# dcherednik/atracdenc

Hardware: AMD Instinct MI355X
Metric: ATRAC3 1024-sample stereo frames/sec (higher is better)
Workload: dtype f32; 1 GPU; ATRAC3 LP2 132 kbps stereo, 64 streams x 64 frames = 4096 frames per GPU per step (BASELINE configs[1]), 'noise' PCM resident in HBM, frames written to HBM (PCIe excluded); streams_per_gpu=64, frame_bytes=384, input=noise, tonal_components=True, parallelism=streams/1, launch=1 process x 1 GPU(s), one host thread and one at3hip context per device, collectives=none (no RCCL); start/stop barrier only

## Files before the change

### atracdenc_amd/csrc/at3_k_backend.hpp

```cpp
#pragma once
#include "at3_bits.hpp"
#include "at3_common.hpp"

namespace at3 {

struct BackParams {
    float* specs;
    const float* ges;
    const Curve* curves;
    PsyRec* psy;
    float* loud;
    float* loud_state;
    uint8_t* out;
    int n_blocks;
    int f0;
    int n_streams;
    int no_tonal;
    int js;
    int frame_sz;
    int bfu_idx_const;
    int mono_js;
    struct QuantRec* quant;
    int flat_literal;
    unsigned long long* counters;
// ... 132 lines not shown
        __syncthreads();
        if (wave > 0) {
            if (k + 2 < kLoudChunks) {
                loud_produce(s_t[k & 1], s_curve, s_ges, u, k + 2, xa);
                if (k + 4 < kLoudChunks) loud_request(p.specs, c0, n_cf, u, k + 4, xa);
            }
        } else if (chain) {
            loud_consume(s_t[(k + 1) & 1] + lane * kLoudRow, l);
        }
        __syncthreads();
    }
    if (chain && c0 + lane < n_cf) p.psy[c0 + lane].loud_ch = l;
}

constexpr int kPsyCf = 4;
__device__ __forceinline__ bool psy_flat_job(int wave, int lane, int& k, int& b)
{
    if (wave == 0) { k = lane / 3; b = 26 + lane % 3; return lane < 12; }
    if (wave == 1) { k = lane / 10; b = 16 + lane % 10; return lane < 40; }
    if (wave == 2) { k = lane / 8; b = 8 + lane % 8; return lane < 32; }
    k = 0; b = 8;
    return false;
}
__device__ __forceinline__ bool psy_scale_job(int wave, int lane, int& k, int& b)
{
    if (wave == 0) { k = lane / 6; b = 26 + lane % 6; return lane < 24; }
    if (wave == 1) { k = lane / 10; b = 16 + lane % 10; return lane < 40; }
    if (wave == 2) { k = lane / 16; b = lane % 16; return true; }
    k = 0; b = 0;
    return false;
}

__device__ __attribute__((noinline)) float flatness_literal_wave(const Libm64* M, const float* sp, int len, double arith, int lane)
{
    const double floor_ = (double)1e-12f;
    double lg = 0.0;
    if (lane < len) {
// ... 34 lines not shown
        float4 x4[kPsyCf];
#pragma unroll
        for (int k = 0; k < kPsyCf; ++k) x4[k] = *reinterpret_cast<const float4*>(specs0 + (size_t)(k < ncf ? k : 0) * 1024 + 4 * tid);
#pragma unroll
        for (int k = 0; k < kPsyCf; ++k) *reinterpret_cast<float4*>(s_spec[k] + 4 * tid) = (k < ncf) ? x4[k] : float4{0.0f, 0.0f, 0.0f, 0.0f};
    }
    if (tid < 32 * kPsyCf) {
        (&s_run_len[0][0])[tid] = 0;
        const int k = tid >> 5, b = tid & 31;
        if (k < ncf && (p.no_tonal || b < 8 || b > 28)) rec0[k].flat[b] = 0.0f;
    }
    if (tid < kPsyCf) s_any[tid] = 0;
    if (tid >= 128 && tid < 192) s_scale[tid - 128] = scale_v;
    __syncthreads();

    int fk, fb;
    const bool flat_job = !p.no_tonal && psy_flat_job(wave, lane, fk, fb) && fk < ncf;
    float flat = 1.0f;
    double arith = 0.0;
    bool want_literal = false;
    if (flat_job) {
        const int b = fb;
        const float* sp = s_spec[fk];
        const int start = bfu_start(b), end = bfu_start(b + 1), len = end - start;
        double prod = 1.0;
        int esum = 0;
        const double floor_ = (double)1e-12f;
        for (int i0 = start; i0 < end; i0 += 8) {
            const float4 xa = *reinterpret_cast<const float4*>(sp + i0), xb = *reinterpret_cast<const float4*>(sp + i0 + 4);
            const float ev[8] = {xa.x * xa.x, xa.y * xa.y, xa.z * xa.z, xa.w * xa.w, xb.x * xb.x, xb.y * xb.y, xb.z * xb.z, xb.w * xb.w};
#pragma unroll
            for (int k = 0; k < 8; ++k) {
                const double e = (double)fmaxf(0.0f, ev[k]);
                arith += e;
                const double d = e > floor_ ? e : floor_;
                const uint64_t bits = (uint64_t)__double_as_longlong(d);
                esum += (int)((bits >> 52) & 0x7ffu) - 1022;
                prod *= __longlong_as_double((long long)((bits & 0x800fffffffffffffull) | 0x3fe0000000000000ull));
            }
        }
        arith /= (double)len;
        if (!(arith <= floor_)) {
            const double meanLog = (log(prod) + (double)esum * 0.69314718055994530942) / (double)len;
            const double ratio = exp(meanLog) / arith;
            const float f_lo = (float)fmin(1.0, fmax(0.0, ratio * (1.0 - 1e-12)));
            const float f_hi = (float)fmin(1.0, fmax(0.0, ratio * (1.0 + 1e-12)));
            flat = f_lo;
            want_literal = f_lo != f_hi || p.flat_literal;
        }
    }
    for (unsigned long long rem = __ballot(want_literal); rem; rem &= rem - 1ull) {
        const int src = __builtin_ctzll(rem);
        const int jk = __builtin_amdgcn_readlane(fk, src), jb = __builtin_amdgcn_readlane(fb, src);
        const uint64_t ab = (uint64_t)__double_as_longlong(arith);
        const uint64_t as = (uint64_t)(uint32_t)__builtin_amdgcn_readlane((int)(uint32_t)ab, src) |
// ... 580 lines not shown
```

### atracdenc_amd/csrc/at3_k_gain.hpp

```cpp
#pragma once
#include "at3_common.hpp"

namespace at3 {

struct GainParams {
    const float* sub;
    GainRec* rec;
    cpx* bins;
    BandState* state;
    Curve* curves;
    int n_blocks;
    int f0;
    int js;
    int n_streams;
    int literal;
};

constexpr int kLowCutBin = 38;

__device__ inline void median3_32(const float* in, float* out)
{
    for (int i = 0; i < 32; ++i) {
        const int lo = i > 0 ? i - 1 : 0;
        const int hi = i < 31 ? i + 1 : 31;
// ... 755 lines not shown
        float m[8] = {ma.x, ma.y, ma.z, ma.w, mb.x, mb.y, mb.z, mb.w};
#pragma unroll
        for (int i = 1; i < 8; ++i) {
#pragma unroll
            for (int k = i; k > 0; --k) {
                const float lo = fminf(m[k - 1], m[k]), hi = fmaxf(m[k - 1], m[k]);
                m[k - 1] = lo;
                m[k] = hi;
            }
        }
        rec->lo[sf] = m[2];
        rec->hi[sf] = m[6];
    }
}

__global__ __launch_bounds__(256) void k_gain_tail(GainParams p, int n_items)
{
    __shared__ float s_g[8][32], s_f[8][32], s_m[8][32];
    const int tid = threadIdx.x, grp = tid >> 5, j = tid & 31, half = grp & 1;
    const int nfr = p.n_blocks - p.f0;
    int item = blockIdx.x * 8 + grp;
    const bool valid = item < n_items;
    if (!valid) item = n_items - 1;
    int wg = item;
    const int band = wg % 3; wg /= 3;
    const int ch = wg % 2; wg /= 2;
    const int f = p.f0 + wg % nfr;
    const int s = wg / nfr;
    GainRec* rec = p.rec + (((size_t)s * p.n_blocks + f) * 2 + ch) * 3 + band;
    const float hfr = rec->hfr;
    const float g_j = rec->gain[j];
    asm volatile("" ::"v"(g_j));
    const bool active = valid && !(hfr < 0.05f);
    if (__ballot(active) == 0ull) return;
    float* s_gain = s_g[grp];
    float* s_filt = s_f[grp];
    float* s_minv = s_m[grp];
    const float in_j = active ? g_j : 0.0f;
    s_gain[j] = in_j;
    wave_sync();
    float filt_j;
    {
        const float a = s_gain[j > 0 ? j - 1 : 0], c = s_gain[j < 31 ? j + 1 : 31];
        if (j == 0) filt_j = fmaxf(in_j, c);
        else if (j == 31) filt_j = fmaxf(a, in_j);
        else filt_j = fmaxf(fminf(a, in_j), fminf(fmaxf(a, in_j), c));
    }
    s_filt[j] = filt_j;
    wave_sync();
    s_minv[j] = (j <= 29) ? fminf(fminf(filt_j, s_filt[j < 30 ? j + 1 : 31]), s_filt[j < 30 ? j + 2 : 31]) : -1.0f;
    wave_sync();
    float maxRaw = 0.0f, sum = 0.0f, bestLevel = 0.0f;
    int bestEnd = -1;
    for (int k = 0; k < 32; ++k) {
        const float g = s_gain[k];
        maxRaw = fmaxf(maxRaw, g);
        sum += g;
        const float mv = s_minv[k];
        if (k <= 29 && mv > bestLevel) {
            bestLevel = mv;
            bestEnd = k + 2;
        }
    }
    const uint32_t ge = (uint32_t)(__ballot(filt_j >= bestLevel) >> (32 * half));
    const uint32_t high = (uint32_t)(__ballot(in_j >= bestLevel * 0.7f) >> (32 * half));
    const float last = s_gain[31];
    float plateau = 0.0f;
    bool release = false;
    if (!(bestLevel < 1e-6f)) {
        plateau = bestLevel;
        const uint32_t x = (bestEnd + 1 < 32) ? (ge >> (bestEnd + 1)) : 0u;
        bestEnd += (x == 0xffffffffu) ? 32 : __builtin_ctz(~x);
        if (bestEnd < 31) {
            if (last < bestLevel * 0.1f) release = true;
            else release = ((high >> (bestEnd + 1)) == 0u) && (last < bestLevel * 0.5f);
        }
    }
    const bool usePlateau = plateau > 1e-6f && !release && plateau >= maxRaw * 0.4f;
    if (active && j == 0) {
        rec->cur_hpf = sum / 32.0f;
        rec->target = usePlateau ? plateau : last;
    }
}

constexpr int kScanChunk = 512;
__global__ __launch_bounds__(64) void k_gain_scan(GainParams p, int n_streams)
{
    __shared__ float s_hfr[kScanChunk], s_g31[kScanChunk], s_tgt[kScanChunk], s_hpf[kScanChunk];
    const int lane = threadIdx.x;
    const int idx = blockIdx.x;
    if (idx >= n_streams * 6) return;
    const int band = idx % 3, ch = (idx / 3) % 2, s = idx / 6;
    BandState* st = p.state + (size_t)s * 8 + ch * 4 + band;
    float lvl = st->last_level, tgt = st->last_target, hpf = st->last_hpf;
    const int nfr = p.n_blocks - p.f0;
    for (int base = 0; base < nfr; base += kScanChunk) {
        const int cnt = (nfr - base < kScanChunk) ? nfr - base : kScanChunk;
        for (int i = lane; i < cnt; i += 64) {
            const GainRec* rec = p.rec + (((size_t)s * p.n_blocks + p.f0 + base + i) * 2 + ch) * 3 + band;
            s_hfr[i] = rec->hfr;
            s_g31[i] = rec->gain[31];
            s_tgt[i] = rec->target;
            s_hpf[i] = rec->cur_hpf;
        }
        __syncthreads();
        if (lane == 0) {
            for (int i = 0; i < cnt; ++i) {
                const float h = s_hfr[i], g = s_g31[i], t = s_tgt[i], e = s_hpf[i];
                s_g31[i] = lvl;
                s_tgt[i] = tgt;
                s_hpf[i] = hpf;
                if (h < 0.05f) {
                    lvl = 0.0f;
                } else {
                    lvl = g;
                    tgt = t;
                    hpf = e;
                }
            }
        }
        __syncthreads();
        for (int i = lane; i < cnt; i += 64) {
            GainRec* rec = p.rec + (((size_t)s * p.n_blocks + p.f0 + base + i) * 2 + ch) * 3 + band;
            rec->ctx_level = s_g31[i];
            rec->ctx_target = s_tgt[i];
            rec->ctx_hpf = s_hpf[i];
        }
        __syncthreads();
    }
    if (lane == 0) {
        st->last_level = lvl;
        st->last_target = tgt;
        st->last_hpf = hpf;
    }
}

__device__ inline uint32_t first_set_bit(uint32_t x)
{
    return x ? 31u - (uint32_t)__builtin_clz(x) : 0u;
}

__device__ inline int relation_to_idx(float x)
{
// ... 18 lines not shown

__device__ __forceinline__ float grp_readlane_f(float v, int idx, int half)
{
    const int a = __builtin_amdgcn_readlane((int)__float_as_uint(v), idx);
    const int b = __builtin_amdgcn_readlane((int)__float_as_uint(v), 32 + idx);
    return __uint_as_float((uint32_t)(half ? b : a));
}
__device__ __forceinline__ int grp_readlane_i(int v, int idx, int half)
{
    const int a = __builtin_amdgcn_readlane(v, idx);
    const int b = __builtin_amdgcn_readlane(v, 32 + idx);
    return half ? b : a;
}

struct CurvePts {
    int n;
    int level[7];
    int loc[7];
};


__device__ __forceinline__ void early_mismatch_score_pair(const Log2fTab* L2, const float* gain_interp, float in_j, float in_next, float target,
                                                          const CurvePts& cpA, const CurvePts& cpB, float* s_tmpA, uint8_t* s_ptsA,
                                                          float* aB, float* sqB, float* ltB, uint8_t* s_ptsB, int j, float& scoreA, float& scoreB)
{
    auto cell_div = [&](const CurvePts& cp) -> float {
        uint64_t lo = (uint64_t)(uint32_t)cp.n, hi = 0;
#pragma unroll
        for (int i = 0; i < 7; ++i) {
            lo |= (uint64_t)((uint32_t)cp.level[i] & 0xffu) << (8 * (i + 1));
            hi |= (uint64_t)((uint32_t)cp.loc[i] & 0xffu) << (8 * i);
        }
        float d[8];
        cell_divisors_packed(lo, hi, gain_interp, 8 * j, d);
        float dsum = 0.0f;
#pragma unroll
        for (int k = 0; k < 8; ++k) dsum += d[k];
        return dsum / 8.0f;
    };
    (void)s_ptsA; (void)s_ptsB;
    const float divA = cell_div(cpA), divB = cell_div(cpB);
    int maxLocA = 0, maxLocB = 0;
#pragma unroll
    for (int i = 0; i < 7; ++i) {
        if (i < cpA.n && cpA.loc[i] > maxLocA) maxLocA = cpA.loc[i];
        if (i < cpB.n && cpB.loc[i] > maxLocB) maxLocB = cpB.loc[i];
    }
    int evalA = maxLocA + 3 > 3 ? maxLocA + 3 : 3, evalB = maxLocB + 3 > 3 ? maxLocB + 3 : 3;
    if (evalA > 32) evalA = 32;
    if (evalB > 32) evalB = 32;
    const float eps = 1e-9f;
    const float modA = in_j / fmaxf(divA, eps), modB = in_j / fmaxf(divB, eps);
    const float eA = at3_log2f(L2, fmaxf(modA, eps) / fmaxf(target, eps)), eB = at3_log2f(L2, fmaxf(modB, eps) / fmaxf(target, eps));
    const float sqA = eA * eA, sqvB = eB * eB;
    const float aA = at3_log2f(L2, fmaxf(divA, eps)), avB = at3_log2f(L2, fmaxf(divB, eps));
    s_tmpA[j] = aA;
    aB[j] = avB;
    wave_sync();
    const float aA_next = s_tmpA[j < 31 ? j + 1 : 31], aB_next = aB[j < 31 ? j + 1 : 31];
    wave_sync();
    const float dA = aA_next - aA, dB = aB_next - avB;
    const float w = 0.5f * (in_j + in_next);
    const float ltermA = dA * dA * w, ltermB = dB * dB * w;
    float* st = s_tmpA + 32;
    st[j] = j < evalA ? sqA : 0.0f;
    st[32 + j] = j + 1 < evalA ? ltermA : 0.0f;
    st[64 + j] = j + 1 < evalA ? w : 0.0f;
    sqB[j] = j < evalB ? sqvB : 0.0f;
    ltB[j] = j + 1 < evalB ? ltermB : 0.0f;
    s_tmpA[j] = j + 1 < evalB ? w : 0.0f;
    wave_sync();
    float fitA = 0.0f, leakA = 0.0f, wsumA = 0.0f, fitB = 0.0f, leakB = 0.0f, wsumB = 0.0f;
    {
        const float4* a4 = reinterpret_cast<const float4*>(st);
        const float4* s4 = reinterpret_cast<const float4*>(sqB);
        const float4* l4 = reinterpret_cast<const float4*>(ltB);
        const float4* w4 = reinterpret_cast<const float4*>(s_tmpA);
#pragma unroll
        for (int q = 0; q < 8; ++q) {
            const float4 va = a4[q], vl = a4[8 + q], vw = a4[16 + q], vb = s4[q], vm = l4[q], vx = w4[q];
            const float v[4] = {va.x, va.y, va.z, va.w};
            const float lt[4] = {vl.x, vl.y, vl.z, vl.w};
            const float ww[4] = {vw.x, vw.y, vw.z, vw.w};
            const float vB[4] = {vb.x, vb.y, vb.z, vb.w};
            const float lB[4] = {vm.x, vm.y, vm.z, vm.w};
            const float wB[4] = {vx.x, vx.y, vx.z, vx.w};
#pragma unroll
            for (int t = 0; t < 4; ++t) {
                fitA += v[t];
                leakA += lt[t];
                wsumA += ww[t];
                fitB += vB[t];
                leakB += lB[t];
                wsumB += wB[t];
            }
        }
    }
    wave_sync();
    fitA /= (float)evalA;
    fitB /= (float)evalB;
    if (wsumA > eps) leakA /= wsumA;
    if (wsumB > eps) leakB /= wsumB;
    scoreA = (target <= 1e-9f) ? 0.0f : fitA + 0.25f * leakA;
    scoreB = (target <= 1e-9f) ? 0.0f : fitB + 0.25f * leakB;
}

__global__ __launch_bounds__(256) void k_gain_curve(GainParams p, const Tables* T, int n_streams)
{
    __shared__ float s_in[8][32];
    __shared__ __attribute__((aligned(16))) float s_filt[8][32];
    __shared__ __attribute__((aligned(16))) float s_tmp[8][128];
    __shared__ __attribute__((aligned(16))) int s_tloc[8][32];
    __shared__ __attribute__((aligned(16))) int s_tdelta[8][32];
    __shared__ int s_tlev[8][32];
    __shared__ uint8_t s_pts[8][16];
    __shared__ uint8_t s_pts2[8][16];
    __shared__ Log2fTab s_l2[4];
    __shared__ float s_gi4[4][32];
    const int tid = threadIdx.x;
    const int grp = tid >> 5, j = tid & 31, half = grp & 1;
    const Log2fTab* L2 = &s_l2[tid >> 6];
    const float* gi = s_gi4[tid >> 6];
    const int nfr = p.n_blocks - p.f0;
    const int n_items = n_streams * nfr * 6;
    int item = blockIdx.x * 8 + grp;
    const bool valid = item < n_items;
    if (!valid) item = n_items - 1;
    int idx = item;
    const int band = idx % 3; idx /= 3;
    const int ch = idx % 2; idx /= 2;
    const int f = p.f0 + idx % nfr;
// ... 15 lines not shown
    {
        const float a = s_in[grp][j > 0 ? j - 1 : 0], c = s_in[grp][j < 31 ? j + 1 : 31];
        if (j == 0) filt_j = fmaxf(in_j, c);
        else if (j == 31) filt_j = fmaxf(a, in_j);
        else filt_j = fmaxf(fminf(a, in_j), fminf(fmaxf(a, in_j), c));
    }
    const float in_next = s_in[grp][j < 31 ? j + 1 : 31];
    s_filt[grp][j] = filt_j;
    float maxGain = fmaxf(0.0f, in_j);
#pragma unroll
    for (int m = 1; m < 32; m <<= 1) maxGain = fmaxf(maxGain, __shfl_xor(maxGain, m, 64));
    wave_sync();

    const bool active = valid && !(hfr < 0.05f) && !(target < 1e-6f) && !(savedLastLevel < 1e-6f);
    if (__ballot(active) == 0ull) {
        if (valid && j == 0) {
            Curve out;
            out.pad = 0;
            out.n = 0;
#pragma unroll
            for (int i = 0; i < 7; ++i) {
                out.level[i] = 0;
                out.loc[i] = 0;
            }
            *dst = out;
        }
        return;
    }
    const float intraRatio = maxGain / fmaxf(target, 1e-9f);
    float interRatio = 1.0f;
    if (prevTarget > 1e-6f) interRatio = fmaxf(prevTarget, target) / fmaxf(fminf(prevTarget, target), 1e-9f);
    const bool sticky = intraRatio <= 7.0f && interRatio <= 10.0f;
    const int raw = relation_to_idx(filt_j / target);
    if (__ballot(active && j <= 30 && raw != 4) == 0ull) {
        if (valid && j == 0) {
            Curve out;
            out.pad = 0;
            out.n = 0;
#pragma unroll
            for (int i = 0; i < 7; ++i) {
                out.level[i] = 0;
                out.loc[i] = 0;
            }
            *dst = out;
        }
        return;
    }
    int minIdx = 0, maxIdx = 0;
    {
        float ratioLo = lo_j / target, ratioHi = hi_j / target;
        if (ratioLo > ratioHi) {
            const float t = ratioLo;
            ratioLo = ratioHi;
            ratioHi = t;
        }
        const int idxLo = relation_to_idx(ratioLo), idxHi = relation_to_idx(ratioHi);
        minIdx = idxLo < idxHi ? idxLo : idxHi;
        maxIdx = idxLo < idxHi ? idxHi : idxLo;
    }
    int L = raw;
// ... 2 lines not shown
        if (__ballot(may_stick) != 0ull) {
            for (int round = 0; round < 32; ++round) {
                const int prev = __builtin_amdgcn_update_dpp(0, L, 0x138, 0xf, 0xf, false);
                const int d = raw - prev;
                const int nl = (may_stick && (d == 1 || d == -1) && prev >= minIdx && prev <= maxIdx) ? prev : raw;
                const bool moved = nl != L;
                L = nl;
                if (__ballot(moved) == 0ull) break;
            }
        }
    }
    const unsigned long long nzm = __ballot(active && j <= 30 && L != 4);
    const uint32_t gm = (uint32_t)(nzm >> (32 * half));
    const int targetSf = gm ? 32 - __builtin_clz(gm) : 0;
    float bs = 1.0f;
    if (j >= 1) {
        float leftMax = 0.0f, rightMax = 0.0f;
        for (int i = (j - 3 > 0 ? j - 3 : 0); i < j; ++i) leftMax = fmaxf(leftMax, s_filt[grp][i]);
        for (int i = j; i < (j + 3 < 32 ? j + 3 : 32); ++i) rightMax = fmaxf(rightMax, s_filt[grp][i]);
        const float eps = 1e-9f;
        bs = fmaxf((rightMax + eps) / (leftMax + eps), (leftMax + eps) / (rightMax + eps));
    }
    int nt = 0;
    {
        int prev = 4;
        uint32_t remaining = targetSf >= 31 ? 0x7fffffffu : ((1u << targetSf) - 1u);
        for (int it = 0; it < 32; ++it) {
            const unsigned long long m = __ballot(L != prev);
            const uint32_t cand = (uint32_t)(m >> (32 * half)) & remaining;
            const bool done = cand == 0u;
            if (__ballot(!done) == 0ull) break;
            const int sf = done ? 0 : 31 - __builtin_clz(cand);
            const int lev = __builtin_amdgcn_ds_bpermute(4 * (32 * half + sf), L);
            const float sc = __uint_as_float((uint32_t)__builtin_amdgcn_ds_bpermute(4 * (32 * half + sf + 1), (int)__float_as_uint(bs)));
            if (!done) {
                const int loc = sf + 1;
// ... 30 lines not shown
            }
        }
        const bool keep_t = has_t && ahead < 6;
        const uint32_t kept = (uint32_t)(__ballot(keep_t) >> (32 * half));
        const int pos = j < 31 ? __popc(kept >> (j + 1)) : 0;
        wave_sync();
        if (keep_t) {
            s_tlev[grp][pos] = my_lev;
            s_tloc[grp][pos] = my_loc;
        }
        nt = __popc(kept);
    }
    wave_sync();
    if (nt > 6) nt = 6;
    CurvePts pts;
    pts.n = (active && targetSf > 0) ? nt : 0;
#pragma unroll
    for (int i = 0; i < 7; ++i) {
        pts.level[i] = (i < pts.n) ? s_tlev[grp][i] : 0;
        pts.loc[i] = (i < pts.n) ? s_tloc[grp][i] : 0;
    }
    const bool have = pts.n > 0;
    if (__ballot(have) == 0ull) {
        if (valid && j == 0) {
            Curve out;
            out.pad = 0;
            out.n = 0;
#pragma unroll
            for (int i = 0; i < 7; ++i) {
                out.level[i] = 0;
                out.loc[i] = 0;
            }
            *dst = out;
        }
        return;
    }

    {
        const int wv = tid >> 6, ln = tid & 63;
        const double l2v = (&T->log2f_tab[0][0])[ln < 36 ? ln : 35];
        const float giv = T->gain_interp[(ln & 31) < 31 ? (ln & 31) : 30];
        if (ln < 36) reinterpret_cast<double*>(&s_l2[wv])[ln] = l2v;
        if (ln < 32) s_gi4[wv][ln] = giv;
        wave_sync();
    }
    if (maxGain < 1e-4f) pts.n = 0;
    if (hfr < 0.3f) pts.n = 0;
    const CurvePts before = pts;
    bool changed = false;
    float hpfRmsNextMod = 0.0f;
    bool validMod = false;
    {
        const int nBefore = (pts.n > 0) ? pts.loc[0] : 32;
        float sum = 0.0f;
        for (int sf = 0; sf < 32; ++sf) {
            const float v = s_in[grp][sf];
            if (sf < nBefore) sum += v;
        }
        if (pts.n > 0 && pts.loc[0] > 0) {
            hpfRmsNextMod = (sum / (float)nBefore) / gain_level_of(pts.level[0]);
            validMod = true;
        } else if (pts.n == 0) {
            hpfRmsNextMod = sum / 32;
            validMod = true;
        }
    }
    const bool p0ok = validMod && prevTarget > 1e-6f && hpfRmsNextMod > 1e-6f;
    if (p0ok) {
        const int p0 = relation_to_idx_hdr(prevTarget / hpfRmsNextMod);
        int it = -1;
#pragma unroll
        for (int i = 6; i >= 0; --i)
            if (i < pts.n && pts.loc[i] == 0) it = i;
        if (it >= 0) {
#pragma unroll
            for (int i = 0; i < 7; ++i)
                if (i == it && pts.level[i] != p0) {
                    pts.level[i] = p0;
                    changed = true;
                }
        } else if (p0 != 4 || pts.n > 0) {
#pragma unroll
            for (int i = 6; i > 0; --i) {
                pts.level[i] = pts.level[i - 1];
                pts.loc[i] = pts.loc[i - 1];
            }
            pts.level[0] = p0;
            pts.loc[0] = 0;
            pts.n++;
            changed = true;
        }
    }
    float scoreBefore, scoreAfter;
    early_mismatch_score_pair(L2, gi, in_j, in_next, target, before, pts, s_tmp[grp], s_pts[grp], s_filt[grp], reinterpret_cast<float*>(s_tloc[grp]),
                              reinterpret_cast<float*>(s_tdelta[grp]), s_pts2[grp], j, scoreBefore, scoreAfter);
    scoreBefore = __uint_as_float((uint32_t)opaque_lane_value((int)__float_as_uint(scoreBefore)));
    scoreAfter = __uint_as_float((uint32_t)opaque_lane_value((int)__float_as_uint(scoreAfter)));
    if (changed) {
        bool keepByBoundary = false;
        if (p0ok) {
            const float x = prevTarget / hpfRmsNextMod;
            const float desired = fminf(fmaxf(x, gain_level_of(15)), gain_level_of(0));
            const float scaleBefore = gain_level_of(before.n == 0 ? 4 : before.level[0]);
            const float scaleAfter = gain_level_of(pts.n == 0 ? 4 : pts.level[0]);
            const float eps = 1e-9f;
            const float errBefore = fabsf(at3_log2f(L2, fmaxf(scaleBefore, eps) / fmaxf(desired, eps)));
            const float errAfter = fabsf(at3_log2f(L2, fmaxf(scaleAfter, eps) / fmaxf(desired, eps)));
            keepByBoundary = (errAfter + 0.20f < errBefore);
        }
        if (!keepByBoundary && scoreAfter > scoreBefore * (1.0f + 0.02f)) pts = before;
    }
    if (pts.n >= 2 && pts.loc[0] == 0 && pts.level[0] == pts.level[1]) {
#pragma unroll
        for (int i = 1; i < 7; ++i) {
            pts.level[i - 1] = pts.level[i];
            pts.loc[i - 1] = pts.loc[i];
        }
        pts.n--;
    }
    if (valid && j == 0) {
        Curve out;
        out.pad = 0;
        out.n = (uint8_t)(have ? pts.n : 0);
#pragma unroll
        for (int i = 0; i < 7; ++i) {
            const bool on = have && i < pts.n;
            out.level[i] = (uint8_t)(on ? pts.level[i] : 0);
            out.loc[i] = (uint8_t)(on ? pts.loc[i] : 0);
        }
        *dst = out;
    }
}

}
```

### atracdenc_amd/csrc/at3hip.hip

```cpp
#include <hip/hip_runtime.h>

#include <stdio.h>
#include <stdlib.h>
#include <string.h>

#include <new>

#include "../../include/at3hip.h"
#include "at3_common.hpp"
#include "at3_host_util.hpp"
#include "at3_k_backend.hpp"
#include "at3_k_alloc.hpp"
#include "at3_k_frontend.hpp"
#include "at3_k_front2.hpp"
#include "at3_k_gain.hpp"

using namespace at3;
using at3host::dev_alloc;
using at3host::fail;

namespace {

const struct {
    uint32_t bitrate;
// ... 1189 lines not shown
    float* d_out = nullptr;
    const size_t nb = (size_t)n * 256 * sizeof(float);
    if (hipMalloc((void**)&d_cv, (size_t)n * sizeof(Curve)) != hipSuccess || hipMalloc((void**)&d_out, 2 * nb) != hipSuccess) return AT3HIP_EDEVICE;
    int rc = AT3HIP_OK;
    if (hipMemcpy(d_cv, curves, (size_t)n * sizeof(Curve), hipMemcpyHostToDevice) != hipSuccess) rc = AT3HIP_EDEVICE;
    if (rc == AT3HIP_OK) {
        hipLaunchKernelGGL(k_debug_cell_divisors, dim3((unsigned)((n + 1) / 2)), dim3(64), 0, c->stream, d_cv, c->d_tables, d_out, d_out + (size_t)n * 256, n);
        if (hipStreamSynchronize(c->stream) != hipSuccess || hipMemcpy(out_packed, d_out, nb, hipMemcpyDeviceToHost) != hipSuccess ||
            hipMemcpy(out_ref, d_out + (size_t)n * 256, nb, hipMemcpyDeviceToHost) != hipSuccess)
            rc = AT3HIP_EDEVICE;
    }
    (void)hipFree(d_cv);
    (void)hipFree(d_out);
    return rc;
}
#endif

#include "at3_decoder_host.hpp"
#include "at3_decode.hpp"

struct at3hip_decoder : at3host::DecoderBase {
    at3hip_decoder_config cfg;
    Dec3Tables* d_tables = nullptr;
    float* d_raw = nullptr;
    Dec3Gains* d_gains = nullptr;
};

namespace {

__attribute__((optnone, noinline)) bool build_dec3_tables(Dec3Tables* t)
// ... 137 lines not shown
```

Before: 15.51 million frames/s.

## Split flatness sums across lanes and replace shared-memory gain reductions with DPP/ballot

Psy flatness computation now splits each band's energy and log-product accumulation into 16-element chunks across several lanes, combines them with DPP row shuffles, and falls back to a serial sum only when the exponent range makes summation order matter. k_gain_tail replaces shared-memory median/min/max scans with lane permutes, DPP max reductions and ballots. k_gain_scan replaces the single-lane serial carry with a ballot-based parallel scan per 64 frames. CurvePts is packed into two 64-bit words to cut register shuffling. The changes aim to reduce serial per-lane work and LDS traffic, at the cost of added complexity and a rounding-sensitive fallback path; a debug kernel for the flat sums is also added.

```diff
diff --git a/atracdenc_amd/csrc/at3_k_backend.hpp b/atracdenc_amd/csrc/at3_k_backend.hpp
--- a/atracdenc_amd/csrc/at3_k_backend.hpp
+++ b/atracdenc_amd/csrc/at3_k_backend.hpp
@@ -170,13 +170,93 @@
 }
 
 constexpr int kPsyCf = 4;
-__device__ __forceinline__ bool psy_flat_job(int wave, int lane, int& k, int& b)
-{
-    if (wave == 0) { k = lane / 3; b = 26 + lane % 3; return lane < 12; }
-    if (wave == 1) { k = lane / 10; b = 16 + lane % 10; return lane < 40; }
-    if (wave == 2) { k = lane / 8; b = 8 + lane % 8; return lane < 32; }
-    k = 0; b = 8;
+__device__ __forceinline__ bool psy_flat_job(int tid, int& k, int& b, int& chunk, int& nch)
+{
+    if (tid < 48) { k = tid / 12; b = 26 + (tid % 12) / 4; chunk = tid % 4; nch = 4; return true; }
+    if (tid < 128) { k = (tid - 48) / 20; b = 16 + ((tid - 48) % 20) / 2; chunk = (tid - 48) % 2; nch = 2; return true; }
+    if (tid < 160) { k = (tid - 128) / 8; b = 8 + (tid - 128) % 8; chunk = 0; nch = 1; return true; }
+    k = 0; b = 8; chunk = 0; nch = 1;
     return false;
+}
+
+struct FlatPart {
+    double arith;
+    double prod;
+    int esum;
+    uint32_t lo, hi;
+};
+__device__ __forceinline__ void flat_part_add(FlatPart& p, float x)
+{
+    const double floor_ = (double)1e-12f;
+    const float ef = fmaxf(0.0f, x * x);
+    const uint32_t fb = __float_as_uint(ef);
+    p.lo = (fb != 0u && fb < p.lo) ? fb : p.lo;
+    p.hi = fb > p.hi ? fb : p.hi;
+    const double e = (double)ef;
+    p.arith += e;
+    const double d = e > floor_ ? e : floor_;
+    const uint64_t bits = (uint64_t)__double_as_longlong(d);
+    p.esum += (int)((bits >> 52) & 0x7ffu) - 1022;
+    p.prod *= __longlong_as_double((long long)((bits & 0x800fffffffffffffull) | 0x3fe0000000000000ull));
+}
+__device__ __forceinline__ FlatPart flat_part16(const float* sp)
+{
+    FlatPart p{0.0, 1.0, 0, 0xffffffffu, 0u};
+#pragma unroll
+    for (int i0 = 0; i0 < 16; i0 += 8) {
+        const float4 xa = *reinterpret_cast<const float4*>(sp + i0), xb = *reinterpret_cast<const float4*>(sp + i0 + 4);
+        const float x[8] = {xa.x, xa.y, xa.z, xa.w, xb.x, xb.y, xb.z, xb.w};
+#pragma unroll
+        for (int k = 0; k < 8; ++k) flat_part_add(p, x[k]);
+    }
+    return p;
+}
+template <int CTRL>
+__device__ __forceinline__ FlatPart flat_part_from(const FlatPart& p)
+{
+    auto f64 = [](double v) {
+        const uint64_t b = (uint64_t)__double_as_longlong(v);
+        const uint32_t lo = (uint32_t)AT3_DPP((uint32_t)b, CTRL, false), hi = (uint32_t)AT3_DPP((uint32_t)(b >> 32), CTRL, false);
+        return __longlong_as_double((long long)(((uint64_t)hi << 32) | lo));
+    };
+    return FlatPart{f64(p.arith), f64(p.prod), (int)AT3_DPP(p.esum, CTRL, false), (uint32_t)AT3_DPP(p.lo, CTRL, false), (uint32_t)AT3_DPP(p.hi, CTRL, false)};
+}
+__device__ __forceinline__ bool flat_sum_is_order_free(uint32_t lo, uint32_t hi, int nch)
+{
+    if (hi == 0u) return true;
+    const int e_max = (int)(hi >> 23) > 1 ? (int)(hi >> 23) : 1, e_min = (int)(lo >> 23) > 1 ? (int)(lo >> 23) : 1;
+    const int log2n = nch == 4 ? 6 : (nch == 2 ? 5 : 4);
+    return e_max < 255 && e_max - e_min <= 29 - log2n;
+}
+__device__ __forceinline__ void flat_sums(const float* sp, int chunk, int nch, double& arith, double& prod, int& esum, bool& split)
+{
+    FlatPart p = flat_part16(sp);
+    const FlatPart q1 = flat_part_from<0x39>(p), q2 = flat_part_from<0x4E>(p), q3 = flat_part_from<0x93>(p);
+    const bool h1 = nch >= 2, h2 = nch == 4;
+    uint32_t lo = p.lo, hi = p.hi;
+    lo = (h1 && q1.lo < lo) ? q1.lo : lo;
+    lo = (h2 && q2.lo < lo) ? q2.lo : lo;
+    lo = (h2 && q3.lo < lo) ? q3.lo : lo;
+    hi = (h1 && q1.hi > hi) ? q1.hi : hi;
+    hi = (h2 && q2.hi > hi) ? q2.hi : hi;
+    hi = (h2 && q3.hi > hi) ? q3.hi : hi;
+    double a = p.arith;
+    a += h1 ? q1.arith : 0.0;
+    a += h2 ? q2.arith : 0.0;
+    a += h2 ? q3.arith : 0.0;
+    prod = p.prod * (h1 ? q1.prod : 1.0) * (h2 ? q2.prod : 1.0) * (h2 ? q3.prod : 1.0);
+    esum = p.esum + (h1 ? q1.esum : 0) + (h2 ? q2.esum : 0) + (h2 ? q3.esum : 0);
+    split = nch == 1 || flat_sum_is_order_free(lo, hi, nch);
+    if (chunk == 0 && !split) {
+        a = 0.0;
+        for (int i0 = 0; i0 < 16 * nch; i0 += 8) {
+            const float4 xa = *reinterpret_cast<const float4*>(sp + i0), xb = *reinterpret_cast<const float4*>(sp + i0 + 4);
+            const float x[8] = {xa.x, xa.y, xa.z, xa.w, xb.x, xb.y, xb.z, xb.w};
+#pragma unroll
+            for (int k = 0; k < 8; ++k) a += (double)fmaxf(0.0f, x[k] * x[k]);
+        }
+    }
+    arith = a;
 }
 __device__ __forceinline__ bool psy_scale_job(int wave, int lane, int& k, int& b)
 {
@@ -241,31 +321,20 @@
     if (tid >= 128 && tid < 192) s_scale[tid - 128] = scale_v;
     __syncthreads();
 
-    int fk, fb;
-    const bool flat_job = !p.no_tonal && psy_flat_job(wave, lane, fk, fb) && fk < ncf;
+    int fk, fb, fchunk, fnch;
+    const bool chunk_job = psy_flat_job(tid, fk, fb, fchunk, fnch);
+    const bool flat_job = !p.no_tonal && chunk_job && fchunk == 0 && fk < ncf;
     float flat = 1.0f;
-    double arith = 0.0;
+    double arith = 0.0, prod = 1.0;
+    int esum = 0;
+    if (!p.no_tonal && wave < 3) {
+        bool split;
+        flat_sums(s_spec[fk] + bfu_start(fb) + 16 * fchunk, fchunk, fnch, arith, prod, esum, split);
+    }
     bool want_literal = false;
     if (flat_job) {
-        const int b = fb;
-        const float* sp = s_spec[fk];
-        const int start = bfu_start(b), end = bfu_start(b + 1), len = end - start;
-        double prod = 1.0;
-        int esum = 0;
+        const int len = 16 * fnch;
         const double floor_ = (double)1e-12f;
-        for (int i0 = start; i0 < end; i0 += 8) {
-            const float4 xa = *reinterpret_cast<const float4*>(sp + i0), xb = *reinterpret_cast<const float4*>(sp + i0 + 4);
-            const float ev[8] = {xa.x * xa.x, xa.y * xa.y, xa.z * xa.z, xa.w * xa.w, xb.x * xb.x, xb.y * xb.y, xb.z * xb.z, xb.w * xb.w};
-#pragma unroll
-            for (int k = 0; k < 8; ++k) {
-                const double e = (double)fmaxf(0.0f, ev[k]);
-                arith += e;
-                const double d = e > floor_ ? e : floor_;
-                const uint64_t bits = (uint64_t)__double_as_longlong(d);
-                esum += (int)((bits >> 52) & 0x7ffu) - 1022;
-                prod *= __longlong_as_double((long long)((bits & 0x800fffffffffffffull) | 0x3fe0000000000000ull));
-            }
-        }
         arith /= (double)len;
         if (!(arith <= floor_)) {
             const double meanLog = (log(prod) + (double)esum * 0.69314718055994530942) / (double)len;
diff --git a/atracdenc_amd/csrc/at3_k_gain.hpp b/atracdenc_amd/csrc/at3_k_gain.hpp
--- a/atracdenc_amd/csrc/at3_k_gain.hpp
+++ b/atracdenc_amd/csrc/at3_k_gain.hpp
@@ -793,10 +793,23 @@
     }
 }
 
+__device__ __forceinline__ float lane_read_f(float v, int src)
+{
+    return __uint_as_float((uint32_t)__builtin_amdgcn_ds_bpermute(4 * src, (int)__float_as_uint(v)));
+}
+__device__ __forceinline__ float half_wave_max(float v, int lane)
+{
+    v = fmaxf(v, __uint_as_float((uint32_t)AT3_DPP(__float_as_uint(v), 0xB1, false)));
+    v = fmaxf(v, __uint_as_float((uint32_t)AT3_DPP(__float_as_uint(v), 0x4E, false)));
+    v = fmaxf(v, __uint_as_float((uint32_t)AT3_DPP(__float_as_uint(v), 0x124, false)));
+    v = fmaxf(v, __uint_as_float((uint32_t)AT3_DPP(__float_as_uint(v), 0x128, false)));
+    return fmaxf(v, lane_read_f(v, lane ^ 16));
+}
+
 __global__ __launch_bounds__(256) void k_gain_tail(GainParams p, int n_items)
 {
-    __shared__ float s_g[8][32], s_f[8][32], s_m[8][32];
-    const int tid = threadIdx.x, grp = tid >> 5, j = tid & 31, half = grp & 1;
+    __shared__ __attribute__((aligned(16))) float s_g[8][32];
+    const int tid = threadIdx.x, grp = tid >> 5, j = tid & 31, half = grp & 1, lane = tid & 63;
     const int nfr = p.n_blocks - p.f0;
     int item = blockIdx.x * 8 + grp;
     const bool valid = item < n_items;
@@ -812,38 +825,40 @@
     asm volatile("" ::"v"(g_j));
     const bool active = valid && !(hfr < 0.05f);
     if (__ballot(active) == 0ull) return;
-    float* s_gain = s_g[grp];
-    float* s_filt = s_f[grp];
-    float* s_minv = s_m[grp];
     const float in_j = active ? g_j : 0.0f;
-    s_gain[j] = in_j;
-    wave_sync();
+    s_g[grp][j] = in_j;
+    const int gl = 32 * half;
     float filt_j;
     {
-        const float a = s_gain[j > 0 ? j - 1 : 0], c = s_gain[j < 31 ? j + 1 : 31];
+        const float a = lane_read_f(in_j, gl + (j > 0 ? j - 1 : 0)), c = lane_read_f(in_j, gl + (j < 31 ? j + 1 : 31));
         if (j == 0) filt_j = fmaxf(in_j, c);
         else if (j == 31) filt_j = fmaxf(a, in_j);
         else filt_j = fmaxf(fminf(a, in_j), fminf(fmaxf(a, in_j), c));
     }
-    s_filt[j] = filt_j;
+    const float f1 = lane_read_f(filt_j, gl + (j < 30 ? j + 1 : 31)), f2 = lane_read_f(filt_j, gl + (j < 30 ? j + 2 : 31));
+    const float mv = (j <= 29) ? fminf(fminf(filt_j, f1), f2) : -1.0f;
+    const float maxRaw = fmaxf(0.0f, half_wave_max(in_j, lane));
+    const float bestLevel = fmaxf(0.0f, half_wave_max(mv, lane));
+    const uint32_t at_best = (uint32_t)(__ballot(j <= 29 && mv == bestLevel) >> (32 * half));
+    int bestEnd = at_best ? __builtin_ctz(at_best) + 2 : -1;
     wave_sync();
-    s_minv[j] = (j <= 29) ? fminf(fminf(filt_j, s_filt[j < 30 ? j + 1 : 31]), s_filt[j < 30 ? j + 2 : 31]) : -1.0f;
-    wave_sync();
-    float maxRaw = 0.0f, sum = 0.0f, bestLevel = 0.0f;
-    int bestEnd = -1;
-    for (int k = 0; k < 32; ++k) {
-        const float g = s_gain[k];
-        maxRaw = fmaxf(maxRaw, g);
-        sum += g;
-        const float mv = s_minv[k];
-        if (k <= 29 && mv > bestLevel) {
-            bestLevel = mv;
-            bestEnd = k + 2;
-        }
+    float sum = 0.0f, last;
+    {
+        const float4* g4 = reinterpret_cast<const float4*>(s_g[grp]);
+        float4 v[8];
+#pragma unroll
+        for (int q = 0; q < 8; ++q) v[q] = g4[q];
+#pragma unroll
+        for (int q = 0; q < 8; ++q) {
+            sum += v[q].x;
+            sum += v[q].y;
+            sum += v[q].z;
+            sum += v[q].w;
+        }
+        last = v[7].w;
     }
     const uint32_t ge = (uint32_t)(__ballot(filt_j >= bestLevel) >> (32 * half));
     const uint32_t high = (uint32_t)(__ballot(in_j >= bestLevel * 0.7f) >> (32 * half));
-    const float last = s_gain[31];
     float plateau = 0.0f;
     bool release = false;
     if (!(bestLevel < 1e-6f)) {
@@ -862,10 +877,8 @@
     }
 }
 
-constexpr int kScanChunk = 512;
 __global__ __launch_bounds__(64) void k_gain_scan(GainParams p, int n_streams)
 {
-    __shared__ float s_hfr[kScanChunk], s_g31[kScanChunk], s_tgt[kScanChunk], s_hpf[kScanChunk];
     const int lane = threadIdx.x;
     const int idx = blockIdx.x;
     if (idx >= n_streams * 6) return;
@@ -873,39 +886,28 @@
     BandState* st = p.state + (size_t)s * 8 + ch * 4 + band;
     float lvl = st->last_level, tgt = st->last_target, hpf = st->last_hpf;
     const int nfr = p.n_blocks - p.f0;
-    for (int base = 0; base < nfr; base += kScanChunk) {
-        const int cnt = (nfr - base < kScanChunk) ? nfr - base : kScanChunk;
-        for (int i = lane; i < cnt; i += 64) {
-            const GainRec* rec = p.rec + (((size_t)s * p.n_blocks + p.f0 + base + i) * 2 + ch) * 3 + band;
-            s_hfr[i] = rec->hfr;
-            s_g31[i] = rec->gain[31];
-            s_tgt[i] = rec->target;
-            s_hpf[i] = rec->cur_hpf;
-        }
-        __syncthreads();
-        if (lane == 0) {
-            for (int i = 0; i < cnt; ++i) {
-                const float h = s_hfr[i], g = s_g31[i], t = s_tgt[i], e = s_hpf[i];
-                s_g31[i] = lvl;
-                s_tgt[i] = tgt;
-                s_hpf[i] = hpf;
-                if (h < 0.05f) {
-                    lvl = 0.0f;
-                } else {
-                    lvl = g;
-                    tgt = t;
-                    hpf = e;
-                }
-            }
-        }
-        __syncthreads();
-        for (int i = lane; i < cnt; i += 64) {
-            GainRec* rec = p.rec + (((size_t)s * p.n_blocks + p.f0 + base + i) * 2 + ch) * 3 + band;
-            rec->ctx_level = s_g31[i];
-            rec->ctx_target = s_tgt[i];
-            rec->ctx_hpf = s_hpf[i];
-        }
-        __syncthreads();
+    for (int base = 0; base < nfr; base += 64) {
+        const int cnt = (nfr - base < 64) ? nfr - base : 64;
+        const bool in = lane < cnt;
+        GainRec* rec = p.rec + (((size_t)s * p.n_blocks + p.f0 + base + (in ? lane : cnt - 1)) * 2 + ch) * 3 + band;
+        const float h = rec->hfr, g = rec->gain[31], t = rec->target, e = rec->cur_hpf;
+        const unsigned long long pass = __ballot(in && !(h < 0.05f));
+        const unsigned long long below = pass & ((1ull << lane) - 1ull);
+        const int src = below ? 63 - __builtin_clzll(below) : lane;
+        const float gp = lane_read_f(g, lane > 0 ? lane - 1 : 0), tp = lane_read_f(t, src), ep = lane_read_f(e, src);
+        const bool prev_passed = lane > 0 && ((pass >> (lane - 1)) & 1ull);
+        if (in) {
+            rec->ctx_level = lane == 0 ? lvl : (prev_passed ? gp : 0.0f);
+            rec->ctx_target = below ? tp : tgt;
+            rec->ctx_hpf = below ? ep : hpf;
+        }
+        if (pass != 0ull) {
+            const int top = 63 - __builtin_clzll(pass);
+            tgt = __uint_as_float((uint32_t)__builtin_amdgcn_readlane((int)__float_as_uint(t), top));
+            hpf = __uint_as_float((uint32_t)__builtin_amdgcn_readlane((int)__float_as_uint(e), top));
+        }
+        const float g_last = __uint_as_float((uint32_t)__builtin_amdgcn_readlane((int)__float_as_uint(g), cnt - 1));
+        lvl = ((pass >> (cnt - 1)) & 1ull) ? g_last : 0.0f;
     }
     if (lane == 0) {
         st->last_level = lvl;
@@ -954,37 +956,32 @@
 }
 
 struct CurvePts {
-    int n;
-    int level[7];
-    int loc[7];
+    uint64_t lo, hi;
+    __device__ __forceinline__ int n() const { return (int)(lo & 0xffu); }
+    __device__ __forceinline__ int level(int i) const { return (int)((lo >> (8 * (i + 1))) & 0xffu); }
+    __device__ __forceinline__ int loc(int i) const { return (int)((hi >> (8 * i)) & 0xffu); }
+    __device__ __forceinline__ void set_n(int n) { lo = (lo & ~0xffull) | (uint64_t)(uint32_t)n; }
 };
 
-
 __device__ __forceinline__ void early_mismatch_score_pair(const Log2fTab* L2, const float* gain_interp, float in_j, float in_next, float target,
-                                                          const CurvePts& cpA, const CurvePts& cpB, float* s_tmpA, uint8_t* s_ptsA,
-                                                          float* aB, float* sqB, float* ltB, uint8_t* s_ptsB, int j, float& scoreA, float& scoreB)
+                                                          const CurvePts& cpA, const CurvePts& cpB, float* s_tmpA,
+                                                          float* aB, float* sqB, float* ltB, int j, int half, float& scoreA, float& scoreB)
 {
     auto cell_div = [&](const CurvePts& cp) -> float {
-        uint64_t lo = (uint64_t)(uint32_t)cp.n, hi = 0;
-#pragma unroll
-        for (int i = 0; i < 7; ++i) {
-            lo |= (uint64_t)((uint32_t)cp.level[i] & 0xffu) << (8 * (i + 1));
-            hi |= (uint64_t)((uint32_t)cp.loc[i] & 0xffu) << (8 * i);
-        }
         float d[8];
-        cell_divisors_packed(lo, hi, gain_interp, 8 * j, d);
+        cell_divisors_packed(cp.lo, cp.hi, gain_interp, 8 * j, d);
         float dsum = 0.0f;
 #pragma unroll
         for (int k = 0; k < 8; ++k) dsum += d[k];
         return dsum / 8.0f;
     };
-    (void)s_ptsA; (void)s_ptsB;
     const float divA = cell_div(cpA), divB = cell_div(cpB);
     int maxLocA = 0, maxLocB = 0;
+    const int nA = cpA.n(), nB = cpB.n();
 #pragma unroll
     for (int i = 0; i < 7; ++i) {
-        if (i < cpA.n && cpA.loc[i] > maxLocA) maxLocA = cpA.loc[i];
-        if (i < cpB.n && cpB.loc[i] > maxLocB) maxLocB = cpB.loc[i];
+        if (i < nA && cpA.loc(i) > maxLocA) maxLocA = cpA.loc(i);
+        if (i < nB && cpB.loc(i) > maxLocB) maxLocB = cpB.loc(i);
     }
     int evalA = maxLocA + 3 > 3 ? maxLocA + 3 : 3, evalB = maxLocB + 3 > 3 ? maxLocB + 3 : 3;
     if (evalA > 32) evalA = 32;
@@ -1010,32 +1007,23 @@
     ltB[j] = j + 1 < evalB ? ltermB : 0.0f;
     s_tmpA[j] = j + 1 < evalB ? w : 0.0f;
     wave_sync();
-    float fitA = 0.0f, leakA = 0.0f, wsumA = 0.0f, fitB = 0.0f, leakB = 0.0f, wsumB = 0.0f;
-    {
-        const float4* a4 = reinterpret_cast<const float4*>(st);
-        const float4* s4 = reinterpret_cast<const float4*>(sqB);
-        const float4* l4 = reinterpret_cast<const float4*>(ltB);
-        const float4* w4 = reinterpret_cast<const float4*>(s_tmpA);
+    float acc = 0.0f;
+    {
+        const int c = j < 6 ? j : 0;
+        const float* list = c < 4 ? s_tmpA + 32 * c : (c == 4 ? sqB : ltB);
+        const float4* l4 = reinterpret_cast<const float4*>(list);
 #pragma unroll
         for (int q = 0; q < 8; ++q) {
-            const float4 va = a4[q], vl = a4[8 + q], vw = a4[16 + q], vb = s4[q], vm = l4[q], vx = w4[q];
-            const float v[4] = {va.x, va.y, va.z, va.w};
-            const float lt[4] = {vl.x, vl.y, vl.z, vl.w};
-            const float ww[4] = {vw.x, vw.y, vw.z, vw.w};
-            const float vB[4] = {vb.x, vb.y, vb.z, vb.w};
-            const float lB[4] = {vm.x, vm.y, vm.z, vm.w};
-            const float wB[4] = {vx.x, vx.y, vx.z, vx.w};
-#pragma unroll
-            for (int t = 0; t < 4; ++t) {
-                fitA += v[t];
-                leakA += lt[t];
-                wsumA += ww[t];
-                fitB += vB[t];
-                leakB += lB[t];
-                wsumB += wB[t];
-            }
-        }
-    }
+            const float4 v = l4[q];
+            acc += v.x;
+            acc += v.y;
+            acc += v.z;
+            acc += v.w;
+        }
+    }
+    const float wsumB = grp_readlane_f(acc, 0, half), wsumA = grp_readlane_f(acc, 3, half);
+    float fitA = grp_readlane_f(acc, 1, half), leakA = grp_readlane_f(acc, 2, half);
+    float fitB = grp_readlane_f(acc, 4, half), leakB = grp_readlane_f(acc, 5, half);
     wave_sync();
     fitA /= (float)evalA;
     fitB /= (float)evalB;
@@ -1045,16 +1033,20 @@
     scoreB = (target <= 1e-9f) ? 0.0f : fitB + 0.25f * leakB;
 }
 
+__device__ __forceinline__ void store_curve(Curve* dst, uint64_t lo, uint64_t hi)
+{
+    static_assert(offsetof(Curve, level) == 1 && offsetof(Curve, loc) == 8, "Curve layout");
+    *reinterpret_cast<uint4*>(dst) = uint4{(uint32_t)lo, (uint32_t)(lo >> 32), (uint32_t)hi, (uint32_t)(hi >> 32)};
+}
+
 __global__ __launch_bounds__(256) void k_gain_curve(GainParams p, const Tables* T, int n_streams)
 {
-    __shared__ float s_in[8][32];
+    __shared__ __attribute__((aligned(16))) float s_in[8][32];
     __shared__ __attribute__((aligned(16))) float s_filt[8][32];
     __shared__ __attribute__((aligned(16))) float s_tmp[8][128];
     __shared__ __attribute__((aligned(16))) int s_tloc[8][32];
     __shared__ __attribute__((aligned(16))) int s_tdelta[8][32];
     __shared__ int s_tlev[8][32];
-    __shared__ uint8_t s_pts[8][16];
-    __shared__ uint8_t s_pts2[8][16];
     __shared__ Log2fTab s_l2[4];
     __shared__ float s_gi4[4][32];
     const int tid = threadIdx.x;
@@ -1100,17 +1092,7 @@
 
     const bool active = valid && !(hfr < 0.05f) && !(target < 1e-6f) && !(savedLastLevel < 1e-6f);
     if (__ballot(active) == 0ull) {
-        if (valid && j == 0) {
-            Curve out;
-            out.pad = 0;
-            out.n = 0;
-#pragma unroll
-            for (int i = 0; i < 7; ++i) {
-                out.level[i] = 0;
-                out.loc[i] = 0;
-            }
-            *dst = out;
-        }
+        if (valid && j == 0) store_curve(dst, 0ull, 0ull);
         return;
     }
     const float intraRatio = maxGain / fmaxf(target, 1e-9f);
@@ -1119,17 +1101,7 @@
     const bool sticky = intraRatio <= 7.0f && interRatio <= 10.0f;
     const int raw = relation_to_idx(filt_j / target);
     if (__ballot(active && j <= 30 && raw != 4) == 0ull) {
-        if (valid && j == 0) {
-            Curve out;
-            out.pad = 0;
-            out.n = 0;
-#pragma unroll
-            for (int i = 0; i < 7; ++i) {
-                out.level[i] = 0;
-                out.loc[i] = 0;
-            }
-            *dst = out;
-        }
+        if (valid && j == 0) store_curve(dst, 0ull, 0ull);
         return;
     }
     int minIdx = 0, maxIdx = 0;
@@ -1162,12 +1134,20 @@
     const uint32_t gm = (uint32_t)(nzm >> (32 * half));
     const int targetSf = gm ? 32 - __builtin_clz(gm) : 0;
     float bs = 1.0f;
-    if (j >= 1) {
+    {
+        const float* fl = s_filt[grp];
+        const float l3 = fl[j >= 3 ? j - 3 : 0], l2 = fl[j >= 2 ? j - 2 : 0], l1 = fl[j >= 1 ? j - 1 : 0];
+        const float r1 = fl[j < 31 ? j + 1 : 31], r2 = fl[j < 30 ? j + 2 : 31];
         float leftMax = 0.0f, rightMax = 0.0f;
-        for (int i = (j - 3 > 0 ? j - 3 : 0); i < j; ++i) leftMax = fmaxf(leftMax, s_filt[grp][i]);
-        for (int i = j; i < (j + 3 < 32 ? j + 3 : 32); ++i) rightMax = fmaxf(rightMax, s_filt[grp][i]);
+        leftMax = fmaxf(leftMax, j >= 3 ? l3 : 0.0f);
+        leftMax = fmaxf(leftMax, j >= 2 ? l2 : 0.0f);
+        leftMax = fmaxf(leftMax, j >= 1 ? l1 : 0.0f);
+        rightMax = fmaxf(rightMax, filt_j);
+        rightMax = fmaxf(rightMax, j < 31 ? r1 : 0.0f);
+        rightMax = fmaxf(rightMax, j < 30 ? r2 : 0.0f);
         const float eps = 1e-9f;
-        bs = fmaxf((rightMax + eps) / (leftMax + eps), (leftMax + eps) / (rightMax + eps));
+        const float v = fmaxf((rightMax + eps) / (leftMax + eps), (leftMax + eps) / (rightMax + eps));
+        bs = j >= 1 ? v : 1.0f;
     }
     int nt = 0;
     {
@@ -1228,25 +1208,20 @@
     wave_sync();
     if (nt > 6) nt = 6;
     CurvePts pts;
-    pts.n = (active && targetSf > 0) ? nt : 0;
-#pragma unroll
-    for (int i = 0; i < 7; ++i) {
-        pts.level[i] = (i < pts.n) ? s_tlev[grp][i] : 0;
-        pts.loc[i] = (i < pts.n) ? s_tloc[grp][i] : 0;
-    }
-    const bool have = pts.n > 0;
+    {
+        const int n = (active && targetSf > 0) ? nt : 0;
+        pts.lo = (uint64_t)(uint32_t)n;
+        pts.hi = 0;
+#pragma unroll
+        for (int i = 0; i < 6; ++i) {
+            const int lev = (i < n) ? s_tlev[grp][i] : 0, loc = (i < n) ? s_tloc[grp][i] : 0;
+            pts.lo |= (uint64_t)((uint32_t)lev & 0xffu) << (8 * (i + 1));
+            pts.hi |= (uint64_t)((uint32_t)loc & 0xffu) << (8 * i);
+        }
+    }
+    const bool have = pts.n() > 0;
     if (__ballot(have) == 0ull) {
-        if (valid && j == 0) {
-            Curve out;
-            out.pad = 0;
-            out.n = 0;
-#pragma unroll
-            for (int i = 0; i < 7; ++i) {
-                out.level[i] = 0;
-                out.loc[i] = 0;
-            }
-            *dst = out;
-        }
+        if (valid && j == 0) store_curve(dst, 0ull, 0ull);
         return;
     }
 
@@ -1258,23 +1233,27 @@
         if (ln < 32) s_gi4[wv][ln] = giv;
         wave_sync();
     }
-    if (maxGain < 1e-4f) pts.n = 0;
-    if (hfr < 0.3f) pts.n = 0;
+    if (maxGain < 1e-4f || hfr < 0.3f) pts.lo = pts.hi = 0;
     const CurvePts before = pts;
     bool changed = false;
     float hpfRmsNextMod = 0.0f;
     bool validMod = false;
     {
-        const int nBefore = (pts.n > 0) ? pts.loc[0] : 32;
+        const int nBefore = (pts.n() > 0) ? pts.loc(0) : 32;
         float sum = 0.0f;
-        for (int sf = 0; sf < 32; ++sf) {
-            const float v = s_in[grp][sf];
-            if (sf < nBefore) sum += v;
-        }
-        if (pts.n > 0 && pts.loc[0] > 0) {
-            hpfRmsNextMod = (sum / (float)nBefore) / gain_level_of(pts.level[0]);
+        const float4* g4 = reinterpret_cast<const float4*>(s_in[grp]);
+#pragma unroll
+        for (int q = 0; q < 8; ++q) {
+            const float4 v = g4[q];
+            sum += (4 * q < nBefore) ? v.x : 0.0f;
+            sum += (4 * q + 1 < nBefore) ? v.y : 0.0f;
+            sum += (4 * q + 2 < nBefore) ? v.z : 0.0f;
+            sum += (4 * q + 3 < nBefore) ? v.w : 0.0f;
+        }
+        if (pts.n() > 0 && pts.loc(0) > 0) {
+            hpfRmsNextMod = (sum / (float)nBefore) / gain_level_of(pts.level(0));
             validMod = true;
-        } else if (pts.n == 0) {
+        } else if (pts.n() == 0) {
             hpfRmsNextMod = sum / 32;
             validMod = true;
         }
@@ -1282,32 +1261,26 @@
     const bool p0ok = validMod && prevTarget > 1e-6f && hpfRmsNextMod > 1e-6f;
     if (p0ok) {
         const int p0 = relation_to_idx_hdr(prevTarget / hpfRmsNextMod);
+        const int n = pts.n();
         int it = -1;
 #pragma unroll
         for (int i = 6; i >= 0; --i)
-            if (i < pts.n && pts.loc[i] == 0) it = i;
+            if (i < n && pts.loc(i) == 0) it = i;
         if (it >= 0) {
-#pragma unroll
-            for (int i = 0; i < 7; ++i)
-                if (i == it && pts.level[i] != p0) {
-                    pts.level[i] = p0;
-                    changed = true;
-                }
-        } else if (p0 != 4 || pts.n > 0) {
-#pragma unroll
-            for (int i = 6; i > 0; --i) {
-                pts.level[i] = pts.level[i - 1];
-                pts.loc[i] = pts.loc[i - 1];
+            if (pts.level(it) != p0) {
+                const int sh = 8 * (it + 1);
+                pts.lo = (pts.lo & ~(0xffull << sh)) | ((uint64_t)(uint32_t)p0 << sh);
+                changed = true;
             }
-            pts.level[0] = p0;
-            pts.loc[0] = 0;
-            pts.n++;
+        } else if (p0 != 4 || n > 0) {
+            pts.lo = ((pts.lo & ~0xffull) << 8) | ((uint64_t)(uint32_t)p0 << 8) | (uint64_t)(uint32_t)(n + 1);
+            pts.hi = pts.hi << 8;
             changed = true;
         }
     }
     float scoreBefore, scoreAfter;
-    early_mismatch_score_pair(L2, gi, in_j, in_next, target, before, pts, s_tmp[grp], s_pts[grp], s_filt[grp], reinterpret_cast<float*>(s_tloc[grp]),
-                              reinterpret_cast<float*>(s_tdelta[grp]), s_pts2[grp], j, scoreBefore, scoreAfter);
+    early_mismatch_score_pair(L2, gi, in_j, in_next, target, before, pts, s_tmp[grp], s_filt[grp], reinterpret_cast<float*>(s_tloc[grp]),
+                              reinterpret_cast<float*>(s_tdelta[grp]), j, half, scoreBefore, scoreAfter);
     scoreBefore = __uint_as_float((uint32_t)opaque_lane_value((int)__float_as_uint(scoreBefore)));
     scoreAfter = __uint_as_float((uint32_t)opaque_lane_value((int)__float_as_uint(scoreAfter)));
     if (changed) {
@@ -1315,8 +1288,8 @@
         if (p0ok) {
             const float x = prevTarget / hpfRmsNextMod;
             const float desired = fminf(fmaxf(x, gain_level_of(15)), gain_level_of(0));
-            const float scaleBefore = gain_level_of(before.n == 0 ? 4 : before.level[0]);
-            const float scaleAfter = gain_level_of(pts.n == 0 ? 4 : pts.level[0]);
+            const float scaleBefore = gain_level_of(before.n() == 0 ? 4 : before.level(0));
+            const float scaleAfter = gain_level_of(pts.n() == 0 ? 4 : pts.level(0));
             const float eps = 1e-9f;
             const float errBefore = fabsf(at3_log2f(L2, fmaxf(scaleBefore, eps) / fmaxf(desired, eps)));
             const float errAfter = fabsf(at3_log2f(L2, fmaxf(scaleAfter, eps) / fmaxf(desired, eps)));
@@ -1324,26 +1297,16 @@
         }
         if (!keepByBoundary && scoreAfter > scoreBefore * (1.0f + 0.02f)) pts = before;
     }
-    if (pts.n >= 2 && pts.loc[0] == 0 && pts.level[0] == pts.level[1]) {
-#pragma unroll
-        for (int i = 1; i < 7; ++i) {
-            pts.level[i - 1] = pts.level[i];
-            pts.loc[i - 1] = pts.loc[i];
-        }
-        pts.n--;
+    if (pts.n() >= 2 && pts.loc(0) == 0 && pts.level(0) == pts.level(1)) {
+        pts.lo = ((pts.lo >> 16) << 8) | (uint64_t)(uint32_t)(pts.n() - 1);
+        pts.hi = pts.hi >> 8;
     }
     if (valid && j == 0) {
-        Curve out;
-        out.pad = 0;
-        out.n = (uint8_t)(have ? pts.n : 0);
-#pragma unroll
-        for (int i = 0; i < 7; ++i) {
-            const bool on = have && i < pts.n;
-            out.level[i] = (uint8_t)(on ? pts.level[i] : 0);
-            out.loc[i] = (uint8_t)(on ? pts.loc[i] : 0);
-        }
-        *dst = out;
-    }
-}
-
-}
+        const int n = have ? pts.n() : 0;
+        const uint64_t keep_lo = n >= 7 ? ~0ull : ((1ull << (8 * (n + 1))) - 1ull);
+        const uint64_t keep_hi = (1ull << (8 * (n < 7 ? n : 7))) - 1ull;
+        store_curve(dst, n > 0 ? pts.lo & keep_lo : 0ull, n > 0 ? pts.hi & keep_hi : 0ull);
+    }
+}
+
+}
diff --git a/atracdenc_amd/csrc/at3hip.hip b/atracdenc_amd/csrc/at3hip.hip
--- a/atracdenc_amd/csrc/at3hip.hip
+++ b/atracdenc_amd/csrc/at3hip.hip
@@ -1227,6 +1227,64 @@
     (void)hipFree(d_out);
     return rc;
 }
+
+namespace {
+__global__ __launch_bounds__(64) void k_debug_flat_sums(const float* lines, int len, double* out_sum, double* out_chain, int32_t* out_split, int n)
+{
+    __shared__ __attribute__((aligned(16))) float s_x[64 * 16];
+    const int lane = threadIdx.x;
+    const int nch = len / 16, per_wave = 64 / nch;
+    const int first = blockIdx.x * per_wave;
+    for (int i = lane; i < 64 * 16; i += 64) {
+        const int bfu = first + i / len;
+        s_x[i] = bfu < n ? lines[(size_t)bfu * len + i % len] : 0.0f;
+    }
+    __syncthreads();
+    const int chunk = lane % nch;
+    double arith, prod;
+    int esum;
+    bool split;
+    flat_sums(s_x + 16 * lane, chunk, nch, arith, prod, esum, split);
+    const int bfu = first + lane / nch;
+    if (chunk == 0 && bfu < n) {
+        double chain = 0.0;
+        const float* x = s_x + 16 * lane;
+        for (int i = 0; i < len; ++i) chain += (double)fmaxf(0.0f, x[i] * x[i]);
+        out_sum[bfu] = arith;
+        out_chain[bfu] = chain;
+        out_split[bfu] = split ? 1 : 0;
+    }
+}
+}
+
+extern "C" __attribute__((visibility("default"))) int at3hip_debug_flat_sums(at3hip_ctx* c, const float* lines, int32_t len, int32_t n, double* out_sum, double* out_chain, int32_t* out_split)
+{
+    if (!c || !lines || (len != 32 && len != 64) || n < 1 || !out_sum || !out_chain || !out_split) return AT3HIP_EINVAL;
+    at3host::DeviceGuard guard(c->device);
+    float* d_x = nullptr;
+    double* d_out = nullptr;
+    int32_t* d_split = nullptr;
+    const size_t xb = (size_t)n * len * sizeof(float), ob = (size_t)n * sizeof(double);
+    if (hipMalloc((void**)&d_x, xb) != hipSuccess || hipMalloc((void**)&d_out, 2 * ob) != hipSuccess || hipMalloc((void**)&d_split, (size_t)n * sizeof(int32_t)) != hipSuccess) {
+        (void)hipFree(d_x);
+        (void)hipFree(d_out);
+        return AT3HIP_EDEVICE;
+    }
+    int rc = AT3HIP_OK;
+    if (hipMemcpy(d_x, lines, xb, hipMemcpyHostToDevice) != hipSuccess) rc = AT3HIP_EDEVICE;
+    if (rc == AT3HIP_OK) {
+        const int per_wave = 64 / (len / 16);
+        hipLaunchKernelGGL(k_debug_flat_sums, dim3((unsigned)((n + per_wave - 1) / per_wave)), dim3(64), 0, c->stream, d_x, (int)len, d_out, d_out + n, d_split, (int)n);
+        if (hipStreamSynchronize(c->stream) != hipSuccess || hipMemcpy(out_sum, d_out, ob, hipMemcpyDeviceToHost) != hipSuccess ||
+            hipMemcpy(out_chain, d_out + n, ob, hipMemcpyDeviceToHost) != hipSuccess ||
+            hipMemcpy(out_split, d_split, (size_t)n * sizeof(int32_t), hipMemcpyDeviceToHost) != hipSuccess)
+            rc = AT3HIP_EDEVICE;
+    }
+    (void)hipFree(d_x);
+    (void)hipFree(d_out);
+    (void)hipFree(d_split);
+    return rc;
+}
 #endif
 
 #include "at3_decoder_host.hpp"
```

New measurement: 15.82 million frames/s (median of 6 runs). 2.0% higher.
